# apache/brpc

Measured on NVIDIA H100. Metric: echo QPS, 1 KB baidu_std, higher is better.
Workload: dtype u8

## Files before the change

### brpc_b200/abi.py

```python
import atexit
import ctypes as C
import gc
import os

import numpy as np

_HERE = os.path.dirname(os.path.abspath(__file__))
lib_path = os.environ.get("B2RPC_LIB") or os.path.join(_HERE, "libb2rpc.so")

B2_OK, B2_E_INVAL, B2_E_NO_DEVICE, B2_E_CUDA, B2_E_CAPACITY, B2_E_NOMEM = 0, -1, -2, -3, -4, -5

RUN_DT = np.dtype([("socket_id", "<u8"), ("offset", "<u4"), ("length", "<u4"),
                   ("preferred_proto", "<i4"), ("flags", "<u4")])
RUN_STATUS_DT = np.dtype([("consumed", "<u4"), ("parse_error", "<u4"), ("n_msgs", "<u4"), ("first_msg", "<u4"),
                          ("preferred_proto", "<i4"), ("n_unanswered", "<u4"), ("resp_off", "<u4"), ("resp_bytes", "<u4")])
H2_FRAME_DT = np.dtype([("type", "u1"), ("flags", "u1"), ("pad", "<u2"), ("stream_id", "<u4"), ("payload_off", "<u4"), ("payload_len", "<u4")])
HPACK_BLOCK_DT = np.dtype([("conn", "<u4"), ("offset", "<u4"), ("length", "<u4"), ("reserved", "<u4")])
H2_RUN_STATUS_DT = np.dtype([("consumed", "<u4"), ("parse_error", "<u4"), ("n_msgs", "<u4"), ("first_msg", "<u4"), ("ctrl_off", "<u4"), ("ctrl_len", "<u4"),
                             ("remote_max_frame_size", "<u4"), ("remote_stream_window_size", "<u4")])
REQUEST_DT = np.dtype([("kind", "<u4"), ("flags", "<u4"), ("method_idx", "<i4"), ("timeout_ms", "<i4"), ("correlation_id", "<i8"), ("log_id", "<i8"),
                       ("compress_type", "<i4"), ("checksum_type", "<i4"), ("frame_type", "<i4"), ("payload_off", "<u4"), ("payload_len", "<u4"),
                       ("attachment_off", "<u4"), ("attachment_len", "<u4"), ("reserved", "<u4")])
REPLY_DT = np.dtype([("flags", "<u4"), ("error_code", "<i4"), ("correlation_id", "<i8"), ("compress_type", "<i4"), ("checksum_type", "<i4"),
                     ("content_type", "<i4"), ("error_text_off", "<u4"), ("error_text_len", "<u4"), ("body_off", "<u4"), ("body_len", "<u4"),
# ... 81 lines not shown
    _fields_ = [("local_consumed", C.c_uint64), ("remote_consumed", C.c_uint64), ("pending_bytes", C.c_uint32), ("flags", C.c_uint32),
                ("error_code", C.c_int32), ("reserved", C.c_uint32)]


class StreamBatchResult(C.Structure):
    _fields_ = [("msgs", C.c_void_p), ("n_msgs", C.c_uint32), ("events", C.c_void_p), ("n_events", C.c_uint32),
                ("out", C.c_void_p), ("out_bytes", C.c_uint32), ("ctrl", C.c_void_p), ("ctrl_bytes", C.c_uint32),
                ("run_ctrl", C.c_void_p), ("n_runs", C.c_uint32)]


REF_DT = np.dtype([("prefix_len", "<u4"), ("src_off", "<u4"), ("src_len", "<u4"), ("reserved", "<u4")])
IOVEC_DT = np.dtype([("base", "<u8"), ("len", "<u8")])
INPUT_COPY, INPUT_PULL, RESP_COPY, RESP_BY_REF, RESP_IOVEC = 0, 1, 0, 1, 2


class B2Error(RuntimeError):
    def __init__(self, code, text):
        super().__init__("b2rpc error %d: %s" % (code, text))
        self.code = code


def _load():
    if not os.path.exists(lib_path):
        raise ImportError("brpc_b200/libb2rpc.so is missing: run `python -c 'import __graft_entry__ as g; g.build()'` "
                          "(nvcc, sm_90a).  There is no CPU fallback.")
    l = C.CDLL(lib_path)
    l.b2_last_error.restype = C.c_char_p
    l.b2_version.restype = C.c_char_p
    l.b2_ctx_create.argtypes = [C.POINTER(Options), C.POINTER(C.c_void_p)]
    l.b2_ctx_destroy.argtypes = [C.c_void_p]
# ... 10 lines not shown
    l.b2_ring_wait.argtypes = [C.c_void_p, C.c_uint32, C.POINTER(BatchResult)]
    l.b2_ring_launches.restype = C.c_uint64; l.b2_ring_launches.argtypes = [C.c_void_p]
    l.b2_ring_phase_ns.argtypes = [C.c_void_p, C.c_uint32, C.c_void_p]
    l.b2_latency_probe.argtypes = [C.c_void_p, C.c_void_p, C.c_uint32, C.c_void_p, C.c_uint32, C.c_uint32, C.c_int, C.c_void_p]
    l.b2_process_batch.argtypes = [C.c_void_p, C.c_void_p, C.c_uint32, C.c_void_p, C.c_uint32, C.POINTER(BatchResult)]
    l.b2_batch_submit.argtypes = [C.c_void_p, C.c_void_p, C.c_uint32, C.c_void_p, C.c_uint32]
    l.b2_batch_collect.argtypes = [C.c_void_p, C.POINTER(BatchResult)]
    l.b2_batch_upload.argtypes = [C.c_void_p, C.c_void_p, C.c_uint32, C.c_void_p, C.c_uint32]
    l.b2_batch_execute.argtypes = [C.c_void_p, C.POINTER(C.c_float), C.POINTER(C.c_uint32)]
    l.b2_batch_execute_many.argtypes = [C.c_void_p, C.c_uint32, C.POINTER(C.c_float), C.POINTER(C.c_uint32)]
    l.b2_batch_launch.argtypes = [C.c_void_p]
    l.b2_batch_wait.argtypes = [C.c_void_p]
    l.b2_elapsed_ms.argtypes = [C.c_void_p, C.c_void_p, C.POINTER(C.c_float)]
    l.b2_batch_download.argtypes = [C.c_void_p, C.POINTER(BatchResult)]
    l.b2_batch_info.argtypes = [C.c_void_p, C.c_void_p]
    l.b2_device_pci_bus_id.argtypes = [C.c_int, C.c_char_p, C.c_int]
    l.b2_stage_times.argtypes = [C.c_void_p, C.POINTER(C.c_char_p), C.POINTER(C.c_float), C.c_int]
    l.b2_crc32c_batch.argtypes = [C.c_void_p, C.c_void_p, C.c_uint32, C.c_void_p, C.c_void_p, C.c_uint32, C.c_void_p]
    l.b2_snappy_uncompress_batch.argtypes = [C.c_void_p, C.c_void_p, C.c_uint32, C.c_void_p, C.c_void_p, C.c_uint32,
                                             C.c_void_p, C.c_uint32, C.c_void_p, C.c_void_p]
    l.b2_snappy_compress_batch.argtypes = [C.c_void_p, C.c_void_p, C.c_uint32, C.c_void_p, C.c_void_p, C.c_uint32,
                                           C.c_void_p, C.c_uint32, C.c_void_p, C.c_void_p]
    l.b2_crc32c_extend.restype = C.c_uint32; l.b2_crc32c_extend.argtypes = [C.c_uint32, C.c_char_p, C.c_size_t]
    l.b2_snappy_max_compressed_length.restype = C.c_size_t; l.b2_snappy_max_compressed_length.argtypes = [C.c_size_t]
    l.b2_snappy_raw_compress.argtypes = [C.c_char_p, C.c_size_t, C.c_void_p, C.POINTER(C.c_size_t)]
    l.b2_snappy_get_uncompressed_length.argtypes = [C.c_char_p, C.c_size_t, C.POINTER(C.c_size_t)]
    l.b2_snappy_raw_uncompress.argtypes = [C.c_char_p, C.c_size_t, C.c_void_p]
    l.b2_hpack_reset.argtypes = [C.c_void_p, C.c_uint32, C.c_uint32]
    l.b2_hpack_decode_batch.argtypes = [C.c_void_p, C.c_void_p, C.c_uint32, C.c_void_p, C.c_uint32, C.c_void_p, C.c_uint32,
                                        C.c_void_p, C.c_void_p, C.c_void_p]
# ... 29 lines not shown
    l.b2_stream_query.argtypes = [C.c_void_p, C.c_int64, C.POINTER(StreamState)]
    l.b2_stream_take_pending.argtypes = [C.c_void_p, C.c_int64, C.c_void_p, C.c_uint32, C.POINTER(C.c_uint32)]
    l.b2_stream_results.argtypes = [C.c_void_p, C.POINTER(StreamBatchResult)]
    l.b2_stream_ring_enable.argtypes = [C.c_void_p, C.c_uint32]
    l.b2_stream_write.argtypes = [C.c_void_p, C.c_void_p, C.c_uint32, C.c_void_p, C.c_uint32, C.c_uint32, C.c_void_p, C.c_uint32, C.c_void_p]
    l.b2_counters_read.argtypes = [C.c_void_p, C.POINTER(C.c_int64)]
    l.b2_counters_device_ptr.restype = C.c_void_p; l.b2_counters_device_ptr.argtypes = [C.c_void_p]
    return l


lib = _load()

ABI_SYMBOLS = ["b2_ctx_create", "b2_ctx_destroy", "b2_last_error", "b2_version", "b2_register_method",
               "b2_set_server_identity", "b2_set_stream_handler", "b2_set_protocols", "b2_block_alloc", "b2_block_free", "b2_block_pool_host_allocs", "b2_set_modes", "b2_ring_start", "b2_ring_stop", "b2_ring_submit", "b2_ring_wait", "b2_ring_launches", "b2_ring_phase_ns", "b2_latency_probe", "b2_process_batch", "b2_batch_submit", "b2_batch_collect", "b2_batch_upload",
               "b2_batch_execute", "b2_batch_execute_many", "b2_batch_download", "b2_batch_launch", "b2_batch_wait",
               "b2_elapsed_ms", "b2_batch_info", "b2_device_pci_bus_id", "b2_stage_times", "b2_crc32c_batch", "b2_crc32c_extend", "b2_snappy_max_compressed_length", "b2_snappy_raw_compress", "b2_snappy_get_uncompressed_length", "b2_snappy_raw_uncompress", "b2_snappy_uncompress_batch", "b2_snappy_compress_batch", "b2_hpack_reset", "b2_hpack_decode_batch", "b2_pack_requests", "b2_pack_responses", "b2_h2_scan_batch", "b2_h2_conn_reset", "b2_h2_configure", "b2_h2_process_batch", "b2_h2_pack_responses", "b2_counters_read",
               "b2_counters_device_ptr", "b2_counters_allreduce", "b2_h2_pack_requests", "b2_h2_conn_set_next_stream_id", "b2_h2_conn_peer_update",
               "b2_h2_client_conn_reset", "b2_h2_client_process_batch", "b2_h2_client_abandon_streams", "b2_h2_conn_set_gunzip",
               "b2_h2_serve_batch", "b2_stream_configure", "b2_stream_open", "b2_stream_set_connected", "b2_stream_close", "b2_stream_query",
               "b2_stream_take_pending", "b2_stream_results", "b2_stream_write", "b2_stream_ring_enable", "b2_h2_ring_enable", "b2_h2_ring_submit",
               "b2_h2_ring_wait", "b2_h2_client_ring_enable", "b2_h2_client_ring_submit", "b2_h2_client_ring_wait"]

ECHO_METHOD = dict(service_full_name=b"example.EchoService", service_name=b"EchoService", method_name=b"Echo",
                   request_type_name=b"example.EchoRequest", handler=1, echo_attachment=1,
                   response_checksum_type=0, response_compress_type=0)


def _check(rc):
    if rc < 0:
        raise B2Error(rc, (lib.b2_last_error() or b"").decode("utf-8", "replace"))
    return rc
# ... 274 lines not shown
                    fm = (writes["flags"] & STREAM_W_FROM_MSG) != 0
                    idx = writes["src_off"][fm].astype(np.int64)
                    lens[fm] = np.where(idx < len(sm), sm["len"][np.minimum(idx, max(len(sm) - 1, 0))] if len(sm) else 0, 0)
                nfr = np.maximum(1, (lens + seg - 1) // seg)
                out_cap = int(((lens + nfr * 38 + 15) // 16 * 16).sum())
            out = np.empty(max(1, out_cap), np.uint8)
        res = np.zeros(n, STREAM_WRITE_RESULT_DT)
        _check(lib.b2_stream_write(self._h, ptr, nb, writes.ctypes.data, n, max_segment_size, out.ctypes.data, out.nbytes, res.ctypes.data))
        return res, out

    def batch_info(self):
        out = (C.c_uint32 * 4)()
        _check(lib.b2_batch_info(self._h, out))
        return {"tile_bytes": out[0], "n_tiles": out[1], "spec_k": out[2], "fused": bool(out[3])}

    def stage_times(self):
        names = (C.c_char_p * 16)()
        ms = (C.c_float * 16)()
        n = lib.b2_stage_times(self._h, names, ms, 16)
        return [(names[i].decode(), ms[i]) for i in range(max(0, min(n, 16)))]

    def crc32c_batch(self, data, offs, lens):
        data = np.ascontiguousarray(data, dtype=np.uint8)
        offs = np.ascontiguousarray(offs, dtype=np.uint32)
        lens = np.ascontiguousarray(lens, dtype=np.uint32)
        out = np.zeros(len(offs), dtype=np.uint32)
        _check(lib.b2_crc32c_batch(self._h, data.ctypes.data, data.nbytes, offs.ctypes.data, lens.ctypes.data,
                                   len(offs), out.ctypes.data))
        return out

# ... 206 lines not shown
```

### brpc_b200/csrc/b2_api.cu

```cuda
#include <cuda_runtime.h>
#include <dlfcn.h>
#include <stdio.h>
#include <time.h>
#include <stdlib.h>
#include <string.h>
#include <algorithm>
#include <mutex>
#include <string>
#include <unordered_map>
#include <vector>
#include "b2_kernels.cuh"
#include "b2_h2.cuh"

using namespace b2;

static thread_local char g_err[512] = "";
static void set_err(const char* fmt, const char* a = "", const char* b = "") { snprintf(g_err, sizeof g_err, fmt, a, b); }

#define CU(call)                                                                          \
    do {                                                                                  \
        cudaError_t e_ = (call);                                                          \
        if (e_ != cudaSuccess) { set_err("%s: %s", #call, cudaGetErrorString(e_)); return B2_E_CUDA; } \
    } while (0)

// ... 6 lines not shown
SmallLayout small_layout(uint32_t nbytes, uint32_t n_runs, uint32_t max_msgs) {
    const uint32_t mb = std::min(std::min(nbytes / 12 + 1, kSmallMsgs), max_msgs), resp = nbytes + mb * 80 + 2048, off_msgs = 64 + n_runs * 32;
    const uint32_t off_refs = off_msgs + mb * 64, off_resp = (off_refs + mb * 16 + 255u) & ~255u;
    return { mb, resp, 64, off_msgs, off_refs, off_resp, off_resp + resp };
}
constexpr uint32_t kSecEvents = 64, kSecMsgs = kSecEvents + kSmallMsgs * 80, kSecCtrl = kSecMsgs + kSmallMsgs * 32,
                   kSecRunCtrl = kSecCtrl + 3 * kStreamCtrlMax * kSmallMsgs, kSecOut = kSecRunCtrl + kSmallRuns * 8;
struct Stage { const char* name; cudaEvent_t ev; };
enum class RingKind { none, batch, batch_streams, h2_server, h2_client };
struct SlotLayout {
    uint64_t end = 256;
    uint32_t add(uint64_t bytes) { const uint64_t off = end; end = (end + bytes + 255u) & ~255ull; return (uint32_t)off; }
};
}

struct b2_ctx {
    b2_options opt;
    DevConfig cfg;
    std::vector<DevMethod> methods;
    uint8_t* d_bytes = nullptr; b2_run* d_runs = nullptr; uint32_t* d_run_tile_base = nullptr;
    TileRec* d_tiles = nullptr; uint32_t* d_tile_base = nullptr; uint32_t* d_tile_scratch = nullptr; uint32_t* d_tile_spec = nullptr; b2_run_status* d_run_status = nullptr;
    uint32_t* d_frame_off = nullptr; uint32_t* d_frame_run = nullptr; b2_msg_desc* d_msgs = nullptr; MsgAux* d_aux = nullptr; PackJob* d_jobs = nullptr; uint32_t* d_slow_idx = nullptr; uint8_t* d_heads = nullptr;
    uint32_t* d_slot = nullptr; uint32_t* d_scan_tmp = nullptr; uint8_t* d_resp = nullptr; uint8_t* d_unz = nullptr; uint16_t* d_snappy_tab = nullptr; HpackState* d_hpack = nullptr; H2Conn* d_h2 = nullptr; H2Stream* d_h2_streams = nullptr; uint8_t* d_h2_slots = nullptr; uint32_t h2_max_conns = B2_H2_MAX_CONNS, h2_pending = B2_H2_MAX_PENDING, h2_stream_bytes = B2_H2_STREAM_BYTES; uint64_t h2_last_in = 0, h2_last_out = 0;
    uint32_t* d_frame_row = nullptr; uint4* d_rows = nullptr;
    std::vector<uint8_t> h2_gunzip; uint8_t* d_h2_gz_merge = nullptr;
    RingKind ring_kind = RingKind::none; RingDev ring_dev = {}; H2RingDev h2r_dev = {}; H2ClientRingDev h2c_dev = {};
    uint8_t* ring_slots = nullptr; volatile uint32_t* ring_ctl = nullptr; uint32_t* d_ring_ticket = nullptr; cudaStream_t ring_stream = nullptr;
    uint32_t ring_next = 1, ring_stride = 0; bool ring_collected[8] = { true, true, true, true, true, true, true, true };
    const void* ring_bytes[8] = {}; const void* ring_pin_base = nullptr; unsigned long long ring_pin_dev = 0; uint64_t ring_launches = 0;
    StreamPass sp_ring = {}; uint8_t* d_st_ring = nullptr; uint32_t ring_next_wait = 1, st_view_ticket = 0;
// ... 14 lines not shown
    b2_run_status* h_run_status = nullptr; b2_msg_desc* h_msgs = nullptr; uint8_t* h_resp = nullptr;
    uint32_t* h_totals = nullptr; uint32_t* h_run_tile_base = nullptr;
    uint32_t n_runs = 0, n_tiles = 0, nbytes = 0, max_run_tiles = 0; uint64_t covered = 0;
    bool uploaded = false, executed = false;
    cudaStream_t stream = nullptr;
    cudaEvent_t ev[kMaxStages + 1];
    const char* stage_names[kMaxStages];
    int n_stages = 0;
    float last_kernel_ms = 0.f; uint32_t last_launches = 0;
    cudaEvent_t ev_first = nullptr, ev_last = nullptr; bool first_pending = true;
    bool profile_stages = false; bool allow_small = true; bool use_fused = true; bool fused_last = false; bool slow_heavy = false;
    bool adaptive_tile = false; bool dense = false; uint32_t avg_frame = 0;
    uint8_t* d_meta = nullptr; uint8_t* h_meta = nullptr;
    uint8_t* d_small = nullptr; uint8_t* h_small = nullptr;
    bool small = false, small_copy_queued = false, use_fused_small = true; SmallLayout sm = {};
};

enum : unsigned { kDevInput = 1, kDevBatch = 2 };
static void overwrites(b2_ctx* c, unsigned what) {
    if (what & kDevInput) { c->h2_last_in = 0; c->h2_last_out = 0; if (c->st_input == c->d_bytes) c->st_input = nullptr; }
    if (what & kDevBatch) { c->uploaded = false; c->executed = false; }
}

static uint32_t g_crc_tab_host[256];
static void crc_table_init() {
    for (uint32_t i = 0; i < 256; i++) {
        uint32_t c = i;
        for (int k = 0; k < 8; k++) c = (c & 1) ? (c >> 1) ^ 0x82f63b78u : (c >> 1);
        g_crc_tab_host[i] = c;
    }
// ... 161 lines not shown
        for (int k = 0; k < 16; k++) for (uint32_t b = 0; b < 256; b++) tab[k * 256 + b] = adv(g_crc_tab_host[b], k);
        for (int j = 0; j < 4; j++) for (uint32_t b = 0; b < 256; b++) tab[(16 + j) * 256 + b] = adv(b << (8 * j), 512);
        for (int t = 0; t < 5; t++) for (int j = 0; j < 4; j++) for (uint32_t b = 0; b < 256; b++)
            tab[kCrcHotWords + (t * 4 + j) * 256 + b] = adv(b << (8 * j), 16 << t);
        CU(cudaMemcpy(c->d_crc_adv, tab.data(), tab.size() * 4, cudaMemcpyHostToDevice));
    }
    CU(cudaFuncSetAttribute(k_resolve, cudaFuncAttributeMaxDynamicSharedMemorySize, 200 * 1024));
    CU(cudaFuncSetAttribute(k_pack_slow<false>, cudaFuncAttributeMaxDynamicSharedMemorySize, (int)(8 * kSnapRing)));
    CU(cudaFuncSetAttribute(k_pack_tma<kPackGroup>, cudaFuncAttributeMaxDynamicSharedMemorySize, (int)(sizeof(PackWarpSmem) * kPackWarps)));
    CU(cudaFuncSetAttribute(k_pack_tma<kPackGroupSmall>, cudaFuncAttributeMaxDynamicSharedMemorySize, (int)(sizeof(PackWarpSmem) * kPackWarps)));
    if (const char* e = getenv("B2_PACK")) c->use_tma_pack = strcmp(e, "reg") != 0;
    if (const char* e = getenv("B2_SMALL")) c->use_fused_small = strcmp(e, "off") != 0;
    if (const char* e = getenv("B2_FUSED")) c->use_fused = strcmp(e, "off") != 0;
    CU(cudaFuncSetAttribute(k_fused, cudaFuncAttributeMaxDynamicSharedMemorySize, (int)(sizeof(FusedWarpSmem) * (kFusedWarps > kFusedWarpsDense ? kFusedWarps : kFusedWarpsDense))));
    CU(cudaFuncSetAttribute(k_small, cudaFuncAttributeMaxDynamicSharedMemorySize, (int)sizeof(SmallSmem)));
    *out = c;
    return B2_OK;
}

extern "C" int b2_set_server_identity(b2_ctx* c, const char* ip_port) {
    if (!c) return B2_E_INVAL;
    if (h2_ring_refuses(c, true)) return B2_E_INVAL;
    const size_t n = ip_port ? strlen(ip_port) : 0;
    if (n >= sizeof c->cfg.identity) { set_err("identity too long"); return B2_E_INVAL; }
    memset(c->cfg.identity, 0, sizeof c->cfg.identity);
    if (n) memcpy(c->cfg.identity, ip_port, n);
    c->cfg.identity_len = (uint32_t)n;
    return B2_OK;
}

// ... 78 lines not shown
        B.resp = c->d_small + c->sm.off_resp;
        B.max_msgs = c->sm.msgs; B.max_resp = c->sm.resp;
    }
    return B;
}

extern "C" int b2_batch_upload(b2_ctx* c, const void* bytes, uint32_t nbytes, const b2_run* runs, uint32_t n_runs) {
    if (!c || (!bytes && nbytes) || (!runs && n_runs)) { set_err("null argument"); return B2_E_INVAL; }
    if (h2_ring_refuses(c, false)) return B2_E_INVAL;
    if ((c->input_mode != B2_INPUT_PULL && nbytes > c->opt.max_batch_bytes) || nbytes >= (1u << 31) || n_runs > c->opt.max_runs) { set_err("batch exceeds ctx capacity"); return B2_E_CAPACITY; }
    uint64_t covered = 0; for (uint32_t r = 0; r < n_runs; r++) covered += runs[r].length;
    if (c->input_mode == B2_INPUT_PULL && covered > c->opt.max_batch_bytes) { set_err("runs exceed ctx capacity"); return B2_E_CAPACITY; }
    c->stream_valid = false; c->st_view_ticket = 0;
    c->covered = covered;
    CU(cudaSetDevice(c->opt.device));
    if (c->adaptive_tile) {
        uint32_t t = 8192;
        const uint32_t per_tile = c->input_mode == B2_INPUT_PULL ? 48u : 6u;
        if (c->input_mode == B2_INPUT_PULL && t < 32768) t = 32768;
        while (t < (1u << 20) && t < per_tile * c->avg_frame) t <<= 1;
        c->cfg.tile_bytes = t; c->cfg.tile_shift = 0; while ((1u << c->cfg.tile_shift) < t) c->cfg.tile_shift++;
    }
    const uint32_t shift = c->cfg.tile_shift, tile = c->cfg.tile_bytes;
    c->dense = tile >= 2048 && c->avg_frame && (uint64_t)c->avg_frame * kSpecK < tile;
    c->cfg.spec_k = c->dense ? kSpecKDense : kSpecK;
    uint64_t nt = 0; uint32_t max_rt = 0;
    for (uint32_t r = 0; r < n_runs; r++) {
        if ((runs[r].offset & 15u) || (uint64_t)runs[r].offset + runs[r].length > nbytes) { set_err("run offset must be 16-aligned and inside the batch"); return B2_E_INVAL; }
        c->h_run_tile_base[r] = (uint32_t)nt;
        const uint32_t t = (uint32_t)(((uint64_t)runs[r].length + tile - 1) >> shift);
// ... 36 lines not shown
    const StreamPass& S = c->sp;
    const uint32_t msg_bound = c->small ? c->sm.msgs : c->opt.max_msgs, sms = c->n_sms;
    CU(cudaMemsetAsync(S.cnts, 0, 4 * (16 + 2 * (size_t)S.cap), s));
    CU(cudaEventRecord(c->st_ev[0], s));
    k_stream_route<<<grid(msg_bound, 256, sms * 4), 256, 0, s>>>(B, S); CU(cudaEventRecord(c->st_ev[1], s));
    k_stream_alloc<<<grid(c->st_max, 256, sms), 256, 0, s>>>(B, S); CU(cudaEventRecord(c->st_ev[2], s));
    k_stream_group<<<grid(msg_bound, 256, sms * 4), 256, 0, s>>>(B, S); CU(cudaEventRecord(c->st_ev[3], s));
    k_stream_run<<<grid(c->st_max, 4, sms * 8), 128, 0, s>>>(B, S); CU(cudaEventRecord(c->st_ev[4], s));
    k_stream_rst<<<grid(c->n_runs, 4, sms * 4), 128, 0, s>>>(B, S); CU(cudaEventRecord(c->st_ev[5], s));
    CU(cudaMemcpyAsync(c->h_st_cnts, S.cnts, 64, cudaMemcpyDeviceToHost, s));
    if (c->ring_kind == RingKind::batch_streams) CU(cudaMemsetAsync(S.cnt, 0, 8 * (size_t)S.cap, s));
    launches += 5; c->stream_ran = true; c->st_input = B.bytes;
    return B2_OK;
}

static int launch_pipeline(b2_ctx* c) {
    const BatchPtrs B = make_ptrs(c);
    DevConfig C = c->cfg;
    const bool fused = c->use_fused && !c->slow_heavy && !c->small && c->input_mode == B2_INPUT_COPY && c->resp_mode == B2_RESP_COPY && c->use_tma_pack &&
                       (((uint64_t)c->nbytes + 255) & ~255ull) + 4096 <= c->opt.max_resp_bytes;
    C.fused = fused ? 1u : 0u; C.ovf_base = (c->nbytes + 255u) & ~255u; c->fused_last = fused;
    cudaStream_t s = c->stream;
    int st = 0; uint32_t launches = 0;
    const bool prof = c->profile_stages;
    auto mark = [&](const char* name) { if (prof) { c->stage_names[st] = name; cudaEventRecord(c->ev[st + 1], s); st++; } };
    const uint32_t mask = c->stage_mask;
    if (mask & 1) CU(cudaMemsetAsync(B.totals, 0, 48, s));
    CU(cudaEventRecord(c->ev[0], s));
    c->stream_ran = false;
    if (c->n_runs == 0) { c->n_stages = 0; c->last_launches = 0; return B2_OK; }
    if (c->small && c->use_fused_small && !prof) {
        k_small<<<1, kSmallThreads, sizeof(SmallSmem), s>>>(B, C);
        launches = 1;
        if (c->stream_armed) { int rc = launch_stream_pass(c, B, s, launches); if (rc != B2_OK) return rc; }
        c->stage_names[0] = "fused_small"; cudaEventRecord(c->ev[1], s);
        c->n_stages = 1; c->last_launches = launches;
        CU(cudaGetLastError());
        return B2_OK;
    }
    const uint32_t sms = c->n_sms;
    if (mask & 1) {
    if (c->n_tiles) {
        k_tile_search<<<(c->n_tiles * 32 + 255) / 256, 256, 0, s>>>(B, C); launches++; mark("tile_search");
        if (C.pull) k_tile_walk_pull<<<(uint32_t)(((uint64_t)c->n_tiles * 8 + 127) / 128), 128, 0, s>>>(B, C);
        else k_tile_walk<<<(c->n_tiles + 127) / 128, 128, 0, s>>>(B, C);
        launches++; mark("tile_walk");
    }
    {
        size_t smem = (size_t)c->max_run_tiles * 12;
        if (smem > 200 * 1024) smem = 0;
        k_resolve<<<c->n_runs, 256, smem, s>>>(B, C, smem == 0 ? 1u : 0u); launches++; mark("resolve");
    }
    if (fused) {
        const uint32_t fw = c->avg_frame && !c->dense ? kFusedWarps : kFusedWarpsDense;
        if (c->n_tiles) { k_fused<<<sms, fw * 32, sizeof(FusedWarpSmem) * fw, s>>>(B, C); launches++; mark("fused"); }
    } else {
    if (c->n_tiles) { k_frame_table<<<(uint32_t)(((uint64_t)c->n_tiles * C.spec_k + 255) / 256), 256, 0, s>>>(B, C); launches++; mark("frame_table"); }
    k_decode<<<sms * B2_DECODE_MIN_BLOCKS, kDecodeWarps * 32, 0, s>>>(B, C); launches++; mark("decode");
    k_scan_blocks<<<sms, kScanBlock, 0, s>>>(B); launches++;
    mark("scan");
    }
    }
    if (fused) {
        if (mask & 4) { k_pack_slow<true><<<sms * B2_SLOW_MIN_BLOCKS, 256, 0, s>>>(B, C); launches++; mark("pack_slow"); }
    } else if (c->use_tma_pack) {
        if (mask & 4) {
            if (c->slow_heavy || c->cfg.by_ref) { C.verify_done = 1; k_crc_verify<<<sms * 6, 256, 0, s>>>(B, C); launches++; mark("crc_verify"); }
            k_pack_slow<false><<<sms * B2_SLOW_MIN_BLOCKS, 256, 8 * kSnapRing, s>>>(B, C); launches++; mark("pack_slow");
        }
        if (mask & 2) {
            if ((c->avg_frame && c->avg_frame < 640) || c->cfg.by_ref) k_pack_tma<kPackGroupSmall><<<sms, kPackWarps * 32, sizeof(PackWarpSmem) * kPackWarps, s>>>(B, C);
            else k_pack_tma<kPackGroup><<<sms, kPackWarps * 32, sizeof(PackWarpSmem) * kPackWarps, s>>>(B, C);
            launches++; mark("pack");
        }
    } else { k_pack<<<sms * B2_PACK_MIN_BLOCKS, 256, 0, s>>>(B, C); launches++; mark("pack"); }
    if (c->resp_mode == B2_RESP_IOVEC && !c->small) {
        k_emit_iov<<<sms * 4, 256, 0, s>>>(B, c->d_iov, (unsigned long long)(uintptr_t)c->h_resp, (unsigned long long)(uintptr_t)c->host_bytes);
        launches++; mark("emit_iov");
    }
    if (c->stream_armed) { int rc = launch_stream_pass(c, B, s, launches); if (rc != B2_OK) return rc; }
    if (!prof) { c->stage_names[0] = "pipeline"; cudaEventRecord(c->ev[1], s); st = 1; }
    c->n_stages = st; c->last_launches = launches;
    CU(cudaGetLastError());
    return B2_OK;
}

static bool replay_refused(const b2_ctx* c) {
    if (!c || !c->uploaded) { set_err("no batch uploaded"); return true; }
    if (c->stream_armed) { set_err("a submitted batch of a context with a stream table must be collected first: this entry point replays a batch and does not run the stream pass"); return true; }
    return false;
}
extern "C" int b2_batch_execute(b2_ctx* c, float* kernel_ms, uint32_t* n_launches) {
    if (replay_refused(c)) return B2_E_INVAL;
    CU(cudaSetDevice(c->opt.device));
    c->profile_stages = true;
    int rc = launch_pipeline(c);
// ... 25 lines not shown
    CU(cudaStreamSynchronize(c->stream));
    float ms = 0.f;
    CU(cudaEventElapsedTime(&ms, e0, e1));
    cudaEventDestroy(e0); cudaEventDestroy(e1);
    c->executed = true;
    if (c->n_stages) { float t = 0.f; cudaEventElapsedTime(&t, c->ev[0], c->ev[c->n_stages]); c->last_kernel_ms = t; }
    if (total_ms) *total_ms = ms;
    if (n_launches) *n_launches = launches;
    return B2_OK;
}

extern "C" int b2_batch_launch(b2_ctx* c) {
    if (replay_refused(c)) return B2_E_INVAL;
    CU(cudaSetDevice(c->opt.device));
    if (c->first_pending) { CU(cudaEventRecord(c->ev_first, c->stream)); c->first_pending = false; }
    int rc = launch_pipeline(c);
    if (rc != B2_OK) return rc;
    CU(cudaEventRecord(c->ev_last, c->stream));
    c->executed = true;
    return B2_OK;
}
extern "C" int b2_batch_wait(b2_ctx* c) {
    if (!c) return B2_E_INVAL;
    CU(cudaSetDevice(c->opt.device));
    CU(cudaStreamSynchronize(c->stream));
    c->first_pending = true;
    return B2_OK;
}
extern "C" int b2_elapsed_ms(b2_ctx* a, b2_ctx* b, float* ms) {
    if (!a || !b || !ms) return B2_E_INVAL;
    CU(cudaSetDevice(a->opt.device));
// ... 628 lines not shown
    if (c->stream_valid && c->stream_ran) {
        for (int i = 0; i < 5; i++, total++) if (total < cap) { names[total] = kStreamStages[i]; float t = 0.f; cudaEventElapsedTime(&t, c->st_ev[i], c->st_ev[i + 1]); ms[total] = t; }
    }
    if (c->sw_ran) {
        for (int i = 0; i < 7; i++, total++) if (total < cap) { names[total] = kSwStages[i]; float t = 0.f; cudaEventElapsedTime(&t, c->sw_ev[i], c->sw_ev[i + 1]); ms[total] = t; }
    }
    return total;
}

extern "C" int b2_batch_info(b2_ctx* c, uint32_t out[4]) {
    if (!c || !out) return B2_E_INVAL;
    out[0] = c->cfg.tile_bytes; out[1] = c->n_tiles; out[2] = c->cfg.spec_k; out[3] = c->fused_last ? 1u : 0u;
    return B2_OK;
}

extern "C" int b2_device_pci_bus_id(int device, char* out, int cap) {
    if (!out || cap < 13) return B2_E_INVAL;
    if (cudaDeviceGetPCIBusId(out, cap, device) != cudaSuccess) { cudaGetLastError(); return B2_E_CUDA; }
    return B2_OK;
}

extern "C" int b2_counters_read(b2_ctx* c, int64_t out[B2_N_COUNTERS]) {
    if (!c || !out) return B2_E_INVAL;
    CU(cudaSetDevice(c->opt.device));
    CU(cudaMemcpy(out, c->d_counters, 8 * B2_N_COUNTERS, cudaMemcpyDeviceToHost));
    return B2_OK;
}
extern "C" void* b2_counters_device_ptr(b2_ctx* c) { return c ? (void*)c->d_counters : nullptr; }
extern "C" int b2_counters_allreduce(b2_ctx* c, void* nccl_comm) {
    if (!c || !nccl_comm) { set_err("null argument"); return B2_E_INVAL; }
// ... 787 lines not shown
```

### brpc_b200/csrc/b2_kernels.cuh

```cuda
#pragma once
#include <cuda_runtime.h>
#include "b2_core.cuh"
#include "b2_inflate.cuh"

namespace b2 {

enum TileKind : uint8_t { kRanOff = 0, kStop = 1, kAmbig = 2 };

struct __align__(16) TileRec {
    uint32_t entry;
    uint32_t exit;
    uint32_t count;
    uint8_t kind;
    int8_t last_proto;
    uint8_t live;
    int8_t pf_in;
};

struct __align__(16) MsgAux {
    uint32_t msg_off;
    uint32_t msg_len;
    uint32_t att_len;
    uint32_t att_off;
    uint32_t cks_off;
// ... 98 lines not shown
    }
};

#if defined(__CUDACC__)

__device__ __forceinline__ uint32_t find_run(const uint32_t* base, uint32_t n_runs, uint32_t tile) {
    uint32_t lo = 0, hi = n_runs;
    while (hi - lo > 1) { const uint32_t mid = (lo + hi) >> 1; if (__ldg(base + mid) <= tile) lo = mid; else hi = mid; }
    return lo;
}
__device__ __forceinline__ bool is_magic(uint32_t w) { return w == kMagicPRPC || w == kMagicSTRM; }
#ifndef B2_SEARCH_FIRST
#define B2_SEARCH_FIRST 2
#endif

__global__ void __launch_bounds__(256, 6) k_tile_search(BatchPtrs B, DevConfig C) {
    const uint32_t warp = (blockIdx.x * blockDim.x + threadIdx.x) >> 5, lane = threadIdx.x & 31;
    if (warp >= B.n_tiles) return;
    const uint4 ti = __ldg(B.tile_info + warp);
    const uint32_t k = ti.z;
    const uint8_t* base = B.bytes + ti.x;
    const uint32_t len = ti.y;
    uint32_t entry = kNone;
    if (k == 0) {
        entry = 0;
    } else {
        const uint32_t t0 = k << C.tile_shift;
        const uint32_t t1 = min(t0 + C.tile_bytes, len);
        for (uint32_t c0 = t0; c0 < t1 && entry == kNone; c0 += (c0 == t0 ? 512u * B2_SEARCH_FIRST : 2048u)) {
            const int nwin = c0 == t0 ? B2_SEARCH_FIRST : 4;
            uint4 v[4]; uint32_t nx[4];
            #pragma unroll
// ... 2089 lines not shown
                uf += 8 + kl + vl;
            }
            *p++ = 0x50; p = put_varint(p, (uint64_t)(long long)R.content_type);
            *p++ = 0x58; p = put_varint(p, (uint64_t)(long long)R.checksum_type);
            *p++ = 0x62; p = put_varint(p, cks_len);
            if (own_cks) p = put_be32(p, crc_be);
            else for (uint32_t k = 0; k < cks_len; k++) *p++ = bytes[R.checksum_value_off + k];
            out_lens[i] = 12 + ml + body_len + att_len;
        }
    }
}

#ifndef B2_SLOW_MIN_BLOCKS
#define B2_SLOW_MIN_BLOCKS 3
#endif
template <bool kLite>
__global__ void __launch_bounds__(256, B2_SLOW_MIN_BLOCKS) k_pack_slow(BatchPtrs B, DevConfig C) {
    const uint32_t lane = threadIdx.x & 31;
    if (B.totals[2] & 3u) return;
    finalize_runs(B, C);
    const uint32_t n_verify = C.verify_done ? 0u : B.totals[7];
    if (B.totals[3] == 0 && n_verify == 0) return;
    __shared__ uint32_t s_hot[kLite ? 1 : kCrcHotWords];
    extern __shared__ __align__(16) uint8_t s_rings[];
    CrcTabs ct; ct.tree = B.crc_adv + kCrcHotWords;
    if (kLite) { ct.hot = B.crc_adv; ct.ring = nullptr; }
    else { crc_tabs_to_smem(s_hot, B.crc_adv); ct.hot = s_hot; ct.ring = s_rings + (threadIdx.x >> 5) * kSnapRing; }
    for (; !C.verify_done;) {
        uint32_t k = 0;
        if (lane == 0) k = atomicAdd(B.totals + 8, 1u);
// ... 781 lines not shown
```

### include/b2rpc.h

```cpp
#ifndef B2RPC_H_
#define B2RPC_H_

#include <stddef.h>
#include <stdint.h>

#ifdef __cplusplus
extern "C" {
#endif

#define B2_OK              0
#define B2_E_INVAL        -1
#define B2_E_NO_DEVICE    -2
#define B2_E_CUDA         -3
#define B2_E_CAPACITY     -4
#define B2_E_NOMEM        -5

#define B2_PARSE_OK                    0
#define B2_PARSE_ERROR_TRY_OTHERS      1
#define B2_PARSE_ERROR_NOT_ENOUGH_DATA 2
#define B2_PARSE_ERROR_TOO_BIG_DATA    3
#define B2_PARSE_ERROR_NO_RESOURCE     4
#define B2_PARSE_ERROR_ABSOLUTELY_WRONG 5

#define B2_PROTOCOL_UNKNOWN       0
// ... 173 lines not shown
int  b2_ring_phase_ns(b2_ctx* ctx, uint32_t ticket, uint64_t out[4]);
int  b2_latency_probe(b2_ctx* ctx, const void* bytes, uint32_t nbytes, const b2_run* runs, uint32_t n_runs,
                      uint32_t iters, int use_ring, float* us_out);

int  b2_batch_upload(b2_ctx* ctx, const void* bytes, uint32_t nbytes,
                     const b2_run* runs, uint32_t n_runs);
int  b2_batch_execute(b2_ctx* ctx, float* kernel_ms, uint32_t* n_launches);
int  b2_batch_download(b2_ctx* ctx, b2_batch_result* out);
int  b2_batch_execute_many(b2_ctx* ctx, uint32_t steps, float* total_ms, uint32_t* n_launches);

int  b2_batch_launch(b2_ctx* ctx);
int  b2_batch_wait(b2_ctx* ctx);
int  b2_elapsed_ms(b2_ctx* a, b2_ctx* b, float* ms);

int  b2_batch_info(b2_ctx* ctx, uint32_t out[4]);

int  b2_device_pci_bus_id(int device, char* out, int cap);

int  b2_stage_times(b2_ctx* ctx, const char** names, float* ms, int cap);

int  b2_crc32c_batch(b2_ctx* ctx, const void* bytes, uint32_t nbytes,
                     const uint32_t* offs, const uint32_t* lens, uint32_t n,
                     uint32_t* out);

int  b2_snappy_uncompress_batch(b2_ctx* ctx, const void* bytes, uint32_t nbytes,
                                const uint32_t* offs, const uint32_t* lens, uint32_t n,
                                void* out, uint32_t out_cap, uint32_t* out_offs, int32_t* out_lens);

int  b2_snappy_compress_batch(b2_ctx* ctx, const void* bytes, uint32_t nbytes,
                              const uint32_t* offs, const uint32_t* lens, uint32_t n,
// ... 289 lines not shown
```

Baseline: 1.013 billion.

## Shrink search and slow-pack blocks, fold totals memset into search, add resident plan

Moves the zeroing of the batch totals from a separate memset into the first block of the tile-search kernel. The search kernel now runs 128-thread blocks on the fused path, and the lite slow-pack kernel runs more, smaller blocks so they can sit beside the resident fused kernel. Adds a residency-planning API that reads per-kernel function attributes and per-SM limits, detects the average frame size from the first run, and drops timing event records on the untimed execute path. The in-kernel zeroing depends on the search kernel running before anything reads the totals, and the smaller blocks change how work is spread across SMs.

```diff
diff --git a/brpc_b200/abi.py b/brpc_b200/abi.py
--- a/brpc_b200/abi.py
+++ b/brpc_b200/abi.py
@@ -119,6 +119,10 @@
 INPUT_COPY, INPUT_PULL, RESP_COPY, RESP_BY_REF, RESP_IOVEC = 0, 1, 0, 1, 2
 
 
+class ResidentKernel(C.Structure):
+    _fields_ = [("name", C.c_char_p), ("regs", C.c_uint32), ("threads", C.c_uint32), ("smem_bytes", C.c_uint32), ("fits", C.c_uint32)]
+
+
 class B2Error(RuntimeError):
     def __init__(self, code, text):
         super().__init__("b2rpc error %d: %s" % (code, text))
@@ -159,6 +163,7 @@
     l.b2_elapsed_ms.argtypes = [C.c_void_p, C.c_void_p, C.POINTER(C.c_float)]
     l.b2_batch_download.argtypes = [C.c_void_p, C.POINTER(BatchResult)]
     l.b2_batch_info.argtypes = [C.c_void_p, C.c_void_p]
+    l.b2_resident_plan.argtypes = [C.c_void_p, C.POINTER(ResidentKernel), C.c_int]
     l.b2_device_pci_bus_id.argtypes = [C.c_int, C.c_char_p, C.c_int]
     l.b2_stage_times.argtypes = [C.c_void_p, C.POINTER(C.c_char_p), C.POINTER(C.c_float), C.c_int]
     l.b2_crc32c_batch.argtypes = [C.c_void_p, C.c_void_p, C.c_uint32, C.c_void_p, C.c_void_p, C.c_uint32, C.c_void_p]
@@ -218,7 +223,7 @@
 ABI_SYMBOLS = ["b2_ctx_create", "b2_ctx_destroy", "b2_last_error", "b2_version", "b2_register_method",
                "b2_set_server_identity", "b2_set_stream_handler", "b2_set_protocols", "b2_block_alloc", "b2_block_free", "b2_block_pool_host_allocs", "b2_set_modes", "b2_ring_start", "b2_ring_stop", "b2_ring_submit", "b2_ring_wait", "b2_ring_launches", "b2_ring_phase_ns", "b2_latency_probe", "b2_process_batch", "b2_batch_submit", "b2_batch_collect", "b2_batch_upload",
                "b2_batch_execute", "b2_batch_execute_many", "b2_batch_download", "b2_batch_launch", "b2_batch_wait",
-               "b2_elapsed_ms", "b2_batch_info", "b2_device_pci_bus_id", "b2_stage_times", "b2_crc32c_batch", "b2_crc32c_extend", "b2_snappy_max_compressed_length", "b2_snappy_raw_compress", "b2_snappy_get_uncompressed_length", "b2_snappy_raw_uncompress", "b2_snappy_uncompress_batch", "b2_snappy_compress_batch", "b2_hpack_reset", "b2_hpack_decode_batch", "b2_pack_requests", "b2_pack_responses", "b2_h2_scan_batch", "b2_h2_conn_reset", "b2_h2_configure", "b2_h2_process_batch", "b2_h2_pack_responses", "b2_counters_read",
+               "b2_elapsed_ms", "b2_batch_info", "b2_resident_plan", "b2_device_pci_bus_id", "b2_stage_times", "b2_crc32c_batch", "b2_crc32c_extend", "b2_snappy_max_compressed_length", "b2_snappy_raw_compress", "b2_snappy_get_uncompressed_length", "b2_snappy_raw_uncompress", "b2_snappy_uncompress_batch", "b2_snappy_compress_batch", "b2_hpack_reset", "b2_hpack_decode_batch", "b2_pack_requests", "b2_pack_responses", "b2_h2_scan_batch", "b2_h2_conn_reset", "b2_h2_configure", "b2_h2_process_batch", "b2_h2_pack_responses", "b2_counters_read",
                "b2_counters_device_ptr", "b2_counters_allreduce", "b2_h2_pack_requests", "b2_h2_conn_set_next_stream_id", "b2_h2_conn_peer_update",
                "b2_h2_client_conn_reset", "b2_h2_client_process_batch", "b2_h2_client_abandon_streams", "b2_h2_conn_set_gunzip",
                "b2_h2_serve_batch", "b2_stream_configure", "b2_stream_open", "b2_stream_set_connected", "b2_stream_close", "b2_stream_query",
@@ -523,6 +528,12 @@
         _check(lib.b2_batch_info(self._h, out))
         return {"tile_bytes": out[0], "n_tiles": out[1], "spec_k": out[2], "fused": bool(out[3])}
 
+    def resident_plan(self):
+        out = (ResidentKernel * 8)()
+        n = _check(lib.b2_resident_plan(self._h, out, 8))
+        return [{"name": out[i].name.decode(), "regs": out[i].regs, "threads": out[i].threads, "smem_bytes": out[i].smem_bytes,
+                 "fits": out[i].fits} for i in range(min(n, 8))]
+
     def stage_times(self):
         names = (C.c_char_p * 16)()
         ms = (C.c_float * 16)()
diff --git a/brpc_b200/csrc/b2_api.cu b/brpc_b200/csrc/b2_api.cu
--- a/brpc_b200/csrc/b2_api.cu
+++ b/brpc_b200/csrc/b2_api.cu
@@ -44,6 +44,7 @@
 };
 }
 
+enum : int { kPlanFused, kPlanSearch, kPlanWalk, kPlanResolve, kPlanSlow, kPlanKernels };
 struct b2_ctx {
     b2_options opt;
     DevConfig cfg;
@@ -88,6 +89,7 @@
     uint8_t* d_meta = nullptr; uint8_t* h_meta = nullptr;
     uint8_t* d_small = nullptr; uint8_t* h_small = nullptr;
     bool small = false, small_copy_queued = false, use_fused_small = true; SmallLayout sm = {};
+    b2_resident_kernel plan[kPlanKernels] = {}; uint32_t sm_regs = 0, sm_smem = 0, sm_warps = 0, sm_blocks = 0, block_smem_reserve = 0;
 };
 
 enum : unsigned { kDevInput = 1, kDevBatch = 2 };
@@ -279,6 +281,25 @@
     if (const char* e = getenv("B2_FUSED")) c->use_fused = strcmp(e, "off") != 0;
     CU(cudaFuncSetAttribute(k_fused, cudaFuncAttributeMaxDynamicSharedMemorySize, (int)(sizeof(FusedWarpSmem) * (kFusedWarps > kFusedWarpsDense ? kFusedWarps : kFusedWarpsDense))));
     CU(cudaFuncSetAttribute(k_small, cudaFuncAttributeMaxDynamicSharedMemorySize, (int)sizeof(SmallSmem)));
+#if defined(__NVCC__)
+    {
+        const void* fn[kPlanKernels] = { (const void*)k_fused, (const void*)k_tile_search, (const void*)k_tile_walk, (const void*)k_resolve, (const void*)k_pack_slow<true> };
+        const char* name[kPlanKernels] = { "k_fused", "k_tile_search", "k_tile_walk", "k_resolve", "k_pack_slow<true>" };
+        const uint32_t threads[kPlanKernels] = { 0, kSearchThreadsFused, 128, 256, kSlowLiteThreads };
+        for (int k = 0; k < kPlanKernels; k++) {
+            cudaFuncAttributes a;
+            CU(cudaFuncGetAttributes(&a, fn[k]));
+            c->plan[k].name = name[k]; c->plan[k].regs = (uint32_t)a.numRegs; c->plan[k].threads = threads[k]; c->plan[k].smem_bytes = (uint32_t)a.sharedSizeBytes;
+        }
+        int v[5] = {};
+        CU(cudaDeviceGetAttribute(&v[0], cudaDevAttrMaxRegistersPerMultiprocessor, o->device));
+        CU(cudaDeviceGetAttribute(&v[1], cudaDevAttrMaxSharedMemoryPerMultiprocessor, o->device));
+        CU(cudaDeviceGetAttribute(&v[2], cudaDevAttrMaxThreadsPerMultiProcessor, o->device));
+        CU(cudaDeviceGetAttribute(&v[3], cudaDevAttrMaxBlocksPerMultiprocessor, o->device));
+        CU(cudaDeviceGetAttribute(&v[4], cudaDevAttrReservedSharedMemoryPerBlock, o->device));
+        c->sm_regs = (uint32_t)v[0]; c->sm_smem = (uint32_t)v[1]; c->sm_warps = (uint32_t)v[2] / 32; c->sm_blocks = (uint32_t)v[3]; c->block_smem_reserve = (uint32_t)v[4];
+    }
+#endif
     *out = c;
     return B2_OK;
 }
@@ -387,6 +408,12 @@
     c->stream_valid = false; c->st_view_ticket = 0;
     c->covered = covered;
     CU(cudaSetDevice(c->opt.device));
+    if (!c->avg_frame && n_runs && runs[0].length >= 12 && (uint64_t)runs[0].offset + 12 <= nbytes) {
+        const uint8_t* f = static_cast<const uint8_t*>(bytes) + runs[0].offset;
+        uint32_t w[2]; memcpy(w, f, 8);
+        const uint32_t body = __builtin_bswap32(w[1]);
+        if ((w[0] == kMagicPRPC || w[0] == kMagicSTRM) && body <= c->cfg.max_body_size && body < (1u << 30)) c->avg_frame = 12 + body;
+    }
     if (c->adaptive_tile) {
         uint32_t t = 8192;
         const uint32_t per_tile = c->input_mode == B2_INPUT_PULL ? 48u : 6u;
@@ -453,7 +480,10 @@
     return B2_OK;
 }
 
-static int launch_pipeline(b2_ctx* c) {
+static uint32_t fused_warps(const b2_ctx* c) { return c->avg_frame && !c->dense ? kFusedWarps : kFusedWarpsDense; }
+static size_t resolve_smem(const b2_ctx* c, bool fused) { const size_t b = (size_t)c->max_run_tiles * 12; return fused || b > 200 * 1024 ? 0 : b; }
+
+static int launch_pipeline(b2_ctx* c, bool timed = true) {
     const BatchPtrs B = make_ptrs(c);
     DevConfig C = c->cfg;
     const bool fused = c->use_fused && !c->slow_heavy && !c->small && c->input_mode == B2_INPUT_COPY && c->resp_mode == B2_RESP_COPY && c->use_tma_pack &&
@@ -464,34 +494,37 @@
     const bool prof = c->profile_stages;
     auto mark = [&](const char* name) { if (prof) { c->stage_names[st] = name; cudaEventRecord(c->ev[st + 1], s); st++; } };
     const uint32_t mask = c->stage_mask;
-    if (mask & 1) CU(cudaMemsetAsync(B.totals, 0, 48, s));
-    CU(cudaEventRecord(c->ev[0], s));
+    const bool small_launch = c->small && c->use_fused_small && !prof;
+    const bool search_zeroes = (mask & 1) && c->n_runs && c->n_tiles && !small_launch;
+    if ((mask & 1) && !search_zeroes) CU(cudaMemsetAsync(B.totals, 0, 48, s));
+    if (timed) CU(cudaEventRecord(c->ev[0], s));
     c->stream_ran = false;
     if (c->n_runs == 0) { c->n_stages = 0; c->last_launches = 0; return B2_OK; }
-    if (c->small && c->use_fused_small && !prof) {
+    if (small_launch) {
         k_small<<<1, kSmallThreads, sizeof(SmallSmem), s>>>(B, C);
         launches = 1;
         if (c->stream_armed) { int rc = launch_stream_pass(c, B, s, launches); if (rc != B2_OK) return rc; }
-        c->stage_names[0] = "fused_small"; cudaEventRecord(c->ev[1], s);
-        c->n_stages = 1; c->last_launches = launches;
+        c->stage_names[0] = "fused_small";
+        if (timed) cudaEventRecord(c->ev[1], s);
+        c->n_stages = timed ? 1 : 0; c->last_launches = launches;
         CU(cudaGetLastError());
         return B2_OK;
     }
     const uint32_t sms = c->n_sms;
     if (mask & 1) {
     if (c->n_tiles) {
-        k_tile_search<<<(c->n_tiles * 32 + 255) / 256, 256, 0, s>>>(B, C); launches++; mark("tile_search");
+        const uint32_t search_threads = fused ? kSearchThreadsFused : 256u;
+        k_tile_search<<<(c->n_tiles * 32 + search_threads - 1) / search_threads, search_threads, 0, s>>>(B, C); launches++; mark("tile_search");
         if (C.pull) k_tile_walk_pull<<<(uint32_t)(((uint64_t)c->n_tiles * 8 + 127) / 128), 128, 0, s>>>(B, C);
         else k_tile_walk<<<(c->n_tiles + 127) / 128, 128, 0, s>>>(B, C);
         launches++; mark("tile_walk");
     }
     {
-        size_t smem = (size_t)c->max_run_tiles * 12;
-        if (smem > 200 * 1024) smem = 0;
+        const size_t smem = resolve_smem(c, fused);
         k_resolve<<<c->n_runs, 256, smem, s>>>(B, C, smem == 0 ? 1u : 0u); launches++; mark("resolve");
     }
     if (fused) {
-        const uint32_t fw = c->avg_frame && !c->dense ? kFusedWarps : kFusedWarpsDense;
+        const uint32_t fw = fused_warps(c);
         if (c->n_tiles) { k_fused<<<sms, fw * 32, sizeof(FusedWarpSmem) * fw, s>>>(B, C); launches++; mark("fused"); }
     } else {
     if (c->n_tiles) { k_frame_table<<<(uint32_t)(((uint64_t)c->n_tiles * C.spec_k + 255) / 256), 256, 0, s>>>(B, C); launches++; mark("frame_table"); }
@@ -501,7 +534,7 @@
     }
     }
     if (fused) {
-        if (mask & 4) { k_pack_slow<true><<<sms * B2_SLOW_MIN_BLOCKS, 256, 0, s>>>(B, C); launches++; mark("pack_slow"); }
+        if (mask & 4) { k_pack_slow<true><<<sms * B2_SLOW_MIN_BLOCKS * (256 / kSlowLiteThreads), kSlowLiteThreads, 0, s>>>(B, C); launches++; mark("pack_slow"); }
     } else if (c->use_tma_pack) {
         if (mask & 4) {
             if (c->slow_heavy || c->cfg.by_ref) { C.verify_done = 1; k_crc_verify<<<sms * 6, 256, 0, s>>>(B, C); launches++; mark("crc_verify"); }
@@ -518,7 +551,7 @@
         launches++; mark("emit_iov");
     }
     if (c->stream_armed) { int rc = launch_stream_pass(c, B, s, launches); if (rc != B2_OK) return rc; }
-    if (!prof) { c->stage_names[0] = "pipeline"; cudaEventRecord(c->ev[1], s); st = 1; }
+    if (!prof && timed) { c->stage_names[0] = "pipeline"; cudaEventRecord(c->ev[1], s); st = 1; }
     c->n_stages = st; c->last_launches = launches;
     CU(cudaGetLastError());
     return B2_OK;
@@ -574,7 +607,7 @@
     if (replay_refused(c)) return B2_E_INVAL;
     CU(cudaSetDevice(c->opt.device));
     if (c->first_pending) { CU(cudaEventRecord(c->ev_first, c->stream)); c->first_pending = false; }
-    int rc = launch_pipeline(c);
+    int rc = launch_pipeline(c, false);
     if (rc != B2_OK) return rc;
     CU(cudaEventRecord(c->ev_last, c->stream));
     c->executed = true;
@@ -1233,6 +1266,36 @@
     return B2_OK;
 }
 
+static uint32_t block_regs(const b2_resident_kernel& k) { return (k.threads + 31) / 32 * ((k.regs * 32 + 255) / 256 * 256); }
+static uint32_t smem_step(uint32_t bytes, uint32_t most) {
+    static const uint32_t kKB[] = { 0, 8, 16, 32, 64, 100, 132, 164, 196, 228 };
+    for (uint32_t kb : kKB) if (kb * 1024 >= bytes) return std::min(kb * 1024, most);
+    return most;
+}
+extern "C" int b2_resident_plan(b2_ctx* c, b2_resident_kernel* out, int cap) {
+    if (!c || (!out && cap > 0)) { set_err("null argument"); return B2_E_INVAL; }
+    if (!c->plan[kPlanFused].name) { set_err("this build has no function attributes to plan with"); return B2_E_INVAL; }
+    b2_resident_kernel k[kPlanKernels];
+    memcpy(k, c->plan, sizeof k);
+    const uint32_t fw = fused_warps(c);
+    k[kPlanFused].threads = fw * 32; k[kPlanFused].smem_bytes += (uint32_t)(sizeof(FusedWarpSmem) * fw);
+    k[kPlanResolve].smem_bytes += (uint32_t)resolve_smem(c, true);
+    const b2_resident_kernel& f = k[kPlanFused];
+    const uint32_t f_regs = block_regs(f), f_smem = f.smem_bytes + c->block_smem_reserve;
+    const uint32_t room_regs = c->sm_regs > f_regs ? c->sm_regs - f_regs : 0, f_step = smem_step(f_smem, c->sm_smem);
+    const uint32_t room_smem = f_step > f_smem ? f_step - f_smem : 0;
+    const uint32_t room_warps = c->sm_warps > fw ? c->sm_warps - fw : 0, room_blocks = c->sm_blocks > 1 ? c->sm_blocks - 1 : 0;
+    for (int i = 0; i < kPlanKernels; i++) {
+        uint32_t n = room_blocks;
+        n = std::min(n, room_regs / std::max(1u, block_regs(k[i])));
+        n = std::min(n, room_smem / (k[i].smem_bytes + c->block_smem_reserve));
+        n = std::min(n, room_warps / ((k[i].threads + 31) / 32));
+        k[i].fits = n;
+    }
+    for (int i = 0; i < kPlanKernels && i < cap; i++) out[i] = k[i];
+    return kPlanKernels;
+}
+
 extern "C" int b2_device_pci_bus_id(int device, char* out, int cap) {
     if (!out || cap < 13) return B2_E_INVAL;
     if (cudaDeviceGetPCIBusId(out, cap, device) != cudaSuccess) { cudaGetLastError(); return B2_E_CUDA; }
diff --git a/brpc_b200/csrc/b2_kernels.cuh b/brpc_b200/csrc/b2_kernels.cuh
--- a/brpc_b200/csrc/b2_kernels.cuh
+++ b/brpc_b200/csrc/b2_kernels.cuh
@@ -136,8 +136,10 @@
 #define B2_SEARCH_FIRST 2
 #endif
 
+constexpr uint32_t kSearchThreadsFused = 128;
 __global__ void __launch_bounds__(256, 6) k_tile_search(BatchPtrs B, DevConfig C) {
     const uint32_t warp = (blockIdx.x * blockDim.x + threadIdx.x) >> 5, lane = threadIdx.x & 31;
+    if (blockIdx.x == 0 && threadIdx.x < 12) B.totals[threadIdx.x] = 0;
     if (warp >= B.n_tiles) return;
     const uint4 ti = __ldg(B.tile_info + warp);
     const uint32_t k = ti.z;
@@ -2257,6 +2259,7 @@
 #ifndef B2_SLOW_MIN_BLOCKS
 #define B2_SLOW_MIN_BLOCKS 3
 #endif
+constexpr uint32_t kSlowLiteThreads = 128;
 template <bool kLite>
 __global__ void __launch_bounds__(256, B2_SLOW_MIN_BLOCKS) k_pack_slow(BatchPtrs B, DevConfig C) {
     const uint32_t lane = threadIdx.x & 31;
diff --git a/include/b2rpc.h b/include/b2rpc.h
--- a/include/b2rpc.h
+++ b/include/b2rpc.h
@@ -211,6 +211,12 @@
 int  b2_elapsed_ms(b2_ctx* a, b2_ctx* b, float* ms);
 
 int  b2_batch_info(b2_ctx* ctx, uint32_t out[4]);
+
+typedef struct b2_resident_kernel {
+    const char* name;
+    uint32_t regs, threads, smem_bytes, fits;
+} b2_resident_kernel;
+int  b2_resident_plan(b2_ctx* ctx, b2_resident_kernel* out, int cap);
 
 int  b2_device_pci_bus_id(int device, char* out, int cap);
 
```

Result: faster. 1.073 billion (median of 6 runs) (+5.9%).
